# m-dayani/EORB_SLAM

Measured on AMD Instinct MI355X. Metric: front-end frames/s (event-accumulate + extract + match) per GPU; HBM GB/s vs roofline, higher is better.
Workload: dtype f32; 1 GPU; BASELINE.json configs[1]: synthetic 1000000 events/slice on 240x180 (shapes generator, DAVIS sensor pixels; raw (x,y,t,p) records resolved on the GPU through the calibrator's undistortion maps built from the EvETHZ intrinsics, as the reference loader does on the CPU), ev2im_gauss sigma=1 -> ORB-1000 (1.2, 4 levels, FAST 10/0, edge 19) -> SearchForInitialization vs previous slice; input=raw, sequences_per_gpu=1, parallelism=1 GPU

## Files before the change

### eorb_slam_amd/csrc/ev_slots.hip

```cpp
#include "eorb_ctx.h"
#include "ev_common.h"
#include "dev_math.h"
#include "sl_hot_asm.h"
#include <algorithm>
#include <memory>
#include <stdlib.h>
#include <string.h>
#include <vector>

namespace eorb {

constexpr uint32_t kNoSlot = 0xffu;
typedef uint16_t slot_entry;
constexpr uint32_t kEntryTag = 0x1000u;
constexpr int kSlotScatWaves = 8;
constexpr uint16_t kNoGeo = 0xffffu;
constexpr int kCountWaves = 16;

__global__ void sl_assign_kernel(const uint32_t* __restrict__ src_info, int nsrc, int W, int H, int h, int TX,
                                 uint32_t* __restrict__ tile_nslots, uint2* __restrict__ slot_tab, uint16_t* __restrict__ slot_geo,
                                 int* __restrict__ info)
{
    const int i = blockIdx.x * blockDim.x + threadIdx.x;
    if (i >= nsrc) { if (i == nsrc) slot_geo[i] = kNoGeo; return; }
// ... 258 lines not shown
                                const int t = (ty0 + dy) * TX + tx0 + dx;
                                const uint32_t o = atomicAdd(&cnt[t >> 1], 1u << (16 * (t & 1)));
                                rk |= (uint64_t)((o >> (16 * (t & 1))) & 0xfffu) << (12 * j);
                            }
                        }
                    }
                    const int k = k0 + u * 64;
                    if (k < cd.n) ((uint64_t*)rec16)[cd.start + k] = (uint64_t)(r16[u] & 0xffffu) | (rk << 16);
                }
                continue;
            }
#pragma unroll
            for (int u = 0; u < U; u++) {
                if (g[u] != kNoGeo) {
                    const int t0 = (int)((g[u] >> 7) & 0x7f) * TX + (int)(g[u] & 0x7f);
                    const bool two_x = (g[u] >> 14) & 1, two_y = (g[u] >> 15) & 1;
                    atomicAdd(&cnt[t0 >> 1], 1u << (16 * (t0 & 1)));
                    if (two_x) atomicAdd(&cnt[(t0 + 1) >> 1], 1u << (16 * ((t0 + 1) & 1)));
                    if (two_y) {
                        atomicAdd(&cnt[(t0 + TX) >> 1], 1u << (16 * ((t0 + TX) & 1)));
                        if (two_x) atomicAdd(&cnt[(t0 + TX + 1) >> 1], 1u << (16 * ((t0 + TX + 1) & 1)));
                    }
                }
            }
        }
        __builtin_amdgcn_wave_barrier();
        uint16_t* sc = segcnt + (size_t)ch * NT;
        const uint16_t* c16 = (const uint16_t*)cnt;
        for (int i = lane; i < NT; i += 64) sc[i] = c16[i];
        __builtin_amdgcn_wave_barrier();
    }
}

__global__ __launch_bounds__(1024) void sl_scan_kernel(const int* __restrict__ slice_chunk0, const uint16_t* __restrict__ segcnt, int NT,
                                                       uint32_t* __restrict__ segbase, uint32_t* __restrict__ tile_cnt,
                                                       uint32_t* __restrict__ tile_base)
{
    __shared__ uint32_t wsum[16];
    __shared__ uint32_t carry;
    const int slice = blockIdx.x;
    const int c0 = slice_chunk0[slice], c1 = slice_chunk0[slice + 1];
    const int lane = threadIdx.x & 63, wave = threadIdx.x >> 6;
    if (threadIdx.x == 0) carry = 0;
    __syncthreads();
    for (int t0 = 0; t0 < NT; t0 += blockDim.x) {
        const int tile = t0 + threadIdx.x;
        uint32_t run = 0;
        if (tile < NT) {
            int c = c0;
            for (; c + 8 <= c1; c += 8) {
                uint32_t v[8];
#pragma unroll
                for (int u = 0; u < 8; u++) v[u] = segcnt[(size_t)(c + u) * NT + tile];
#pragma unroll
                for (int u = 0; u < 8; u++) { segbase[(size_t)(c + u) * NT + tile] = run; run += v[u]; }
            }
            for (; c < c1; c++) { const uint32_t v = segcnt[(size_t)c * NT + tile]; segbase[(size_t)c * NT + tile] = run; run += v; }
            tile_cnt[(size_t)slice * NT + tile] = run;
        }
        const uint32_t padded = (run + 15u) & ~15u;
        uint32_t incl = (uint32_t)wave_incl_scan((int)padded);
        if (lane == 63) wsum[wave] = incl;
        __syncthreads();
        uint32_t before = carry;
        for (int w = 0; w < wave; w++) before += wsum[w];
        if (tile < NT) tile_base[(size_t)slice * NT + tile] = before + incl - padded;
        __syncthreads();
        if (threadIdx.x == blockDim.x - 1) carry = before + incl;
        __syncthreads();
    }
}

__global__ __launch_bounds__(64 * kSlotScatWaves) void sl_scatter_kernel(const eorb_raw_event* __restrict__ ev, const ChunkDesc* __restrict__ chunks,
                                                                         const uint2* __restrict__ slot_tab, int stride, int LW, int LH, int TX, int TY,
                                                                         int NT, int chunk_cap, const int64_t* __restrict__ slice_ebase,
                                                                         const uint32_t* __restrict__ segbase, const uint32_t* __restrict__ tile_base,
                                                                         slot_entry* __restrict__ entries)
{
    extern __shared__ unsigned char sm2[];
    __shared__ uint32_t s_wsum[kSlotScatWaves];
    constexpr int NTHR = 64 * kSlotScatWaves;
    constexpr int R = 2;
    const int tid = threadIdx.x, lane = tid & 63, wave = tid >> 6;
    const int chunk = blockIdx.x;
    const ChunkDesc cd = chunks[chunk];
    const int NTp = (NT + 1) & ~1;
    uint32_t* pay = (uint32_t*)sm2;
    uint16_t* prng = (uint16_t*)(pay + chunk_cap);
    uint16_t* sidx = prng + chunk_cap;
    uint16_t* cntw = sidx + (size_t)chunk_cap * R * R;
    uint16_t* loff = cntw + kSlotScatWaves * NTp;
    uint32_t* gbase = (uint32_t*)(loff + NTp + 2);
// ... 881 lines not shown
            const int g = std::min(ncu, (nchunks + kCountWaves - 1) / kCountWaves);
            static const int tc_env = [] { const char* e = getenv("EORB_SLOT_TRANSCODE"); return e ? atoi(e) : 1; }();
            uint16_t* d_rec16 = nullptr;
            static const int pre_env = [] { const char* e = getenv("EORB_SLOT_PRERANK"); return e ? atoi(e) : 1; }();
            const int pre_on = c->dbg_slot_prerank >= 0 ? c->dbg_slot_prerank : pre_env;
            if (pre_on && (stride == 16 || stride == 4 || stride == 2) && nsrc <= 65535 && sc.rank && sl_lds_pre(NT, chunk) <= 158 * 1024) {
                if ((rc = ensure(c, ws.rec16, sizeof(uint64_t) * (size_t)std::max<int64_t>(h_offsets[B], 1)))) return rc;
                d_rec16 = (uint16_t*)ws.rec16.p;
                prerank = true;
#define SL_COUNTR(ST, BIT) do { if ((rc = sl_optin(c, BIT, (const void*)sl_count_lds_kernel<ST, false, true>, 159 * 1024))) return rc; \
                sl_count_lds_kernel<ST, false, true><<<g, 64 * kCountWaves, lds_c, M>>>(d_ev, d_chunks, nchunks, d_geo, c->lut_w, c->lut_h, TX, NT, d_segcnt, SlotDict{nullptr, 0u, nullptr, nullptr, 0}, d_rec16); } while (0)
                if (stride == 16) SL_COUNTR(16, 18); else if (stride == 4) SL_COUNTR(4, 19); else SL_COUNTR(2, 20);
#undef SL_COUNTR
            }
            else {
            if (tc_env && stride == 16 && nsrc <= 65535 && sc.rank) {
                if ((rc = ensure(c, ws.rec16, sizeof(uint16_t) * (size_t)std::max<int64_t>(h_offsets[B], 1)))) return rc;
                d_rec16 = (uint16_t*)ws.rec16.p;
            }
#define SL_COUNT(ST, BIT) do { if ((rc = sl_optin(c, BIT, (const void*)sl_count_lds_kernel<ST>, 159 * 1024))) return rc; \
                sl_count_lds_kernel<ST><<<g, 64 * kCountWaves, lds_c, M>>>(d_ev, d_chunks, nchunks, d_geo, c->lut_w, c->lut_h, TX, NT, d_segcnt, SlotDict{nullptr, 0u, nullptr, nullptr}, d_rec16); } while (0)
            if (stride == 16) SL_COUNT(16, 0); else if (stride == 4) SL_COUNT(4, 1); else if (stride == 2) SL_COUNT(2, 10); else SL_COUNT(-4, 2);
#undef SL_COUNT
            if (d_rec16) { d_ev = (const eorb_raw_event*)d_rec16; scat_stride = 2; }
            }
        }
        else if (nchunks) {
            if (stride == 16) sl_count_kernel<16><<<nchunks, 256, lds, M>>>(d_ev, d_chunks, d_tab, c->lut_w, c->lut_h, TX, NT, d_segcnt);
            else if (stride == 4) sl_count_kernel<4><<<nchunks, 256, lds, M>>>(d_ev, d_chunks, d_tab, c->lut_w, c->lut_h, TX, NT, d_segcnt);
            else if (stride == 2) sl_count_kernel<2><<<nchunks, 256, lds, M>>>(d_ev, d_chunks, d_tab, c->lut_w, c->lut_h, TX, NT, d_segcnt);
            else sl_count_kernel<-4><<<nchunks, 256, lds, M>>>(d_ev, d_chunks, d_tab, c->lut_w, c->lut_h, TX, NT, d_segcnt);
        }
        ps.reset(); ps.reset(new ProfScope(c, "ev_scan"));
        sl_scan_kernel<<<B, 1024, 0, M>>>(d_slice_c0, d_segcnt, NT, d_segbase, d_tile_cnt, d_tile_base);
        ps.reset();
        EORB_HIP(c, hipEventRecord(E[0], M));
        EORB_HIP(c, hipStreamWaitEvent(P, E[0], 0));
        EORB_HIP(c, hipMemsetAsync(ws.hot.p, 0, 256, P));
        sl_plan_kernel<<<NT, 256, sizeof(uint32_t) * 2 * (size_t)B, P>>>(d_tile_cnt, d_tile_base, d_slice_eb, B, NT, TX, hot_min, d_nslots, d_rowbase,
                                                                               d_items, d_tile_w, d_tile_m, d_ctr, d_hot_cnt, d_hot_items, hot_cap);
        sl_tasks_kernel<<<1, 1024, sizeof(uint32_t) * (size_t)NT, P>>>(d_tile_w, d_tile_m, NT, Gt, max_per_tile, d_scr, d_task, d_hot_cnt, hot_cap);
        EORB_HIP(c, hipEventRecord(E[1], P));
        ProfScope ps2(c, "ev_scatter");
        const int stride = scat_stride;
        if (nchunks && prerank) {
            const size_t lds_p = sl_lds_pre(NT, chunk);
            const uint16_t* d_segcnt_c = d_segcnt;
            if (sc.waves == 16) {
                if ((rc = sl_optin(c, 16, (const void*)sl_scatter_pre_kernel<16>, 159 * 1024))) return rc;
                sl_scatter_pre_kernel<16><<<nchunks, 64 * 16, lds_p, M>>>((const uint64_t*)ws.rec16.p, d_chunks, d_tab, c->lut_w * c->lut_h, TX, NT, chunk, d_slice_eb, d_segcnt_c, d_segbase, d_tile_base, (slot_entry*)ws.entries.p);
            } else {
                if ((rc = sl_optin(c, 17, (const void*)sl_scatter_pre_kernel<8>, 159 * 1024))) return rc;
                sl_scatter_pre_kernel<8><<<nchunks, 64 * 8, lds_p, M>>>((const uint64_t*)ws.rec16.p, d_chunks, d_tab, c->lut_w * c->lut_h, TX, NT, chunk, d_slice_eb, d_segcnt_c, d_segbase, d_tile_base, (slot_entry*)ws.entries.p);
            }
        }
        else if (nchunks && sc.rank) {
#define SL_SCAT(ST, NW, BIT) do { if ((rc = sl_optin(c, BIT, (const void*)sl_scatter_rank_kernel<ST, NW>, 159 * 1024))) return rc; \
                sl_scatter_rank_kernel<ST, NW><<<nchunks, 64 * NW, sc.lds, M>>>(d_ev, d_chunks, d_tab, c->lut_w, c->lut_h, TX, NT, chunk, \
                                                                                   d_slice_eb, d_segbase, d_tile_base, (slot_entry*)ws.entries.p); } while (0)
            if (sc.waves == 16) { if (stride == 16) SL_SCAT(16, 16, 3); else if (stride == 4) SL_SCAT(4, 16, 4); else if (stride == 2) SL_SCAT(2, 16, 11); else SL_SCAT(-4, 16, 5); }
            else { if (stride == 16) SL_SCAT(16, 8, 6); else if (stride == 4) SL_SCAT(4, 8, 7); else if (stride == 2) SL_SCAT(2, 8, 12); else SL_SCAT(-4, 8, 8); }
#undef SL_SCAT
        }
        else if (nchunks)
            sl_scatter_kernel<<<nchunks, 64 * kSlotScatWaves, sc.lds, M>>>(d_ev, d_chunks, d_tab, stride, c->lut_w, c->lut_h, TX, TY, NT, chunk,
                                                                                 d_slice_eb, d_segbase, d_tile_base, (slot_entry*)ws.entries.p);
        EORB_LAUNCH_CHECK(c, "ev_bin (slot) kernels");
// ... 77 lines not shown
```

### eorb_slam_amd/csrc/orb_extract.hip

```cpp
#include "eorb_ctx.h"
#include "dev_math.h"
#include "orb_pattern.h"
#include <math.h>
#include <algorithm>
#include <string.h>
#include <vector>

namespace eorb {

struct DevGeom {
    LevelGeom lv[kMaxLevels];
    int nlevels, edge, W, H;
    int pyr_bytes, roi_bytes, ncells, cell_cap, cand_total, kp_total, max_out;
    int iniTh, minTh;
    int umax[16];
    float sf[kMaxLevels];
    int oct_in_lds[2][7], oct_off[2][7];
    int oct_lds_bytes[2], oct_gblock_bytes[2];
    int oct_dyn[2], oct_off_dyn[2][7], oct_dyn_base[2], oct_dyn_lds[2];
    int oct_direct_cap[2];
    int node_cap_max, vsp_cap_max, ncap_max;
};

__device__ __constant__ signed char c_pattern[1024];
// ... 53 lines not shown
    }
}

__global__ void pyr_resize_kernel(int level, const DevGeom* __restrict__ G, const short4* __restrict__ tabs,
                                  uint8_t* __restrict__ pyr)
{
    const LevelGeom& L = G->lv[level];
    const LevelGeom& P = G->lv[level - 1];
    const int slice = blockIdx.y;
    uint8_t* base = pyr + (size_t)slice * G->pyr_bytes;
    const uint8_t* sroi = base + P.buf_off + (size_t)G->edge * P.bw + G->edge;
    uint8_t* dst = base + L.buf_off;
    const short4* xt = tabs + L.xtab_off;
    const short4* yt = tabs + L.ytab_off;
    const int n = L.bw * L.bh;
    for (int i = blockIdx.x * blockDim.x + threadIdx.x; i < n; i += gridDim.x * blockDim.x) {
        const int y = i / L.bw, x = i - y * L.bw;
        const int dy = reflect101(y - G->edge, L.h), dx = reflect101(x - G->edge, L.w);
        const short4 xc = xt[dx], yc = yt[dy];
        const uint8_t* S0 = sroi + (size_t)yc.x * P.bw;
        const uint8_t* S1 = sroi + (size_t)yc.y * P.bw;
        int r0, r1;
        if (dx < L.xmax) {
            r0 = S0[xc.x] * xc.y + S0[xc.x + 1] * xc.z;
            r1 = S1[xc.x] * xc.y + S1[xc.x + 1] * xc.z;
        } else {
            r0 = S0[xc.x] * 2048;
            r1 = S1[xc.x] * 2048;
        }
        dst[i] = (uint8_t)((((yc.z * (r0 >> 4)) >> 16) + ((yc.w * (r1 >> 4)) >> 16) + 2) >> 2);
    }
}

__device__ __forceinline__ int fast_S(const uint8_t* __restrict__ t, int pitch)
{
    const int v = t[0];
    int d[16];
    d[0] = v - t[3 * pitch];          d[1] = v - t[3 * pitch + 1];   d[2] = v - t[2 * pitch + 2];   d[3] = v - t[pitch + 3];
    d[4] = v - t[3];                  d[5] = v - t[-pitch + 3];      d[6] = v - t[-2 * pitch + 2];  d[7] = v - t[-3 * pitch + 1];
    d[8] = v - t[-3 * pitch];         d[9] = v - t[-3 * pitch - 1];  d[10] = v - t[-2 * pitch - 2]; d[11] = v - t[-pitch - 3];
    d[12] = v - t[-3];                d[13] = v - t[pitch - 3];      d[14] = v - t[2 * pitch - 2];  d[15] = v - t[3 * pitch - 1];
    int mn2[16], mx2[16], mn4[16], mx4[16], mn8[16], mx8[16];
#pragma unroll
    for (int k = 0; k < 16; k++) { mn2[k] = min(d[k], d[(k + 1) & 15]); mx2[k] = max(d[k], d[(k + 1) & 15]); }
#pragma unroll
    for (int k = 0; k < 16; k++) { mn4[k] = min(mn2[k], mn2[(k + 2) & 15]); mx4[k] = max(mx2[k], mx2[(k + 2) & 15]); }
#pragma unroll
    for (int k = 0; k < 16; k++) { mn8[k] = min(mn4[k], mn4[(k + 4) & 15]); mx8[k] = max(mx4[k], mx4[(k + 4) & 15]); }
    int A = -256, Bm = 256;
#pragma unroll
    for (int k = 0; k < 16; k++) {
        A = max(A, min(mn8[k], d[(k + 8) & 15]));
        Bm = min(Bm, max(mx8[k], d[(k + 8) & 15]));
    }
    return max(A, -Bm);
}

constexpr int kCellMax = 60;

__global__ __launch_bounds__(256) void fast_cells_kernel(const DevGeom* __restrict__ G, const uint8_t* __restrict__ pyr,
                                                         int32_t* __restrict__ cell_cnt, uint32_t* __restrict__ cell_cand)
{
    __shared__ uint8_t tile[(kCellMax + 6) * (kCellMax + 8)];
    __shared__ uint8_t smap[(kCellMax + 2) * (kCellMax + 2)];
    __shared__ uint8_t s_cnt[16 * 4];
    const int slice = blockIdx.y;
    int cid = blockIdx.x, level = 0;
    while (level + 1 < G->nlevels && cid >= G->lv[level + 1].cell_off) level++;
    const LevelGeom& L = G->lv[level];
    const int local = cid - L.cell_off;
    const int ci = local / L.nCols, cj = local - ci * L.nCols;
    const int tid = threadIdx.x;
    int32_t* out_cnt = cell_cnt + (size_t)slice * G->ncells + cid;
    uint32_t* out = cell_cand + ((size_t)slice * G->ncells + cid) * G->cell_cap;
    const int iniY = L.minBY + ci * L.hCell, iniX = L.minBX + cj * L.wCell;
    int maxY = iniY + L.hCell + 6, maxX = iniX + L.wCell + 6;
    if (iniY >= L.maxBY - 3 || iniX >= L.maxBX - 3) { if (tid == 0) *out_cnt = 0; return; }
    maxY = min(maxY, L.maxBY); maxX = min(maxX, L.maxBX);
    const int cw = maxX - iniX, ch = maxY - iniY;
    const int dw = cw - 6, dh = ch - 6;
    if (dw <= 0 || dh <= 0) { if (tid == 0) *out_cnt = 0; return; }
    const uint8_t* roi = pyr + (size_t)slice * G->pyr_bytes + L.buf_off + (size_t)G->edge * L.bw + G->edge;
    const int pitch = kCellMax + 8;
    const uint8_t first = roi[(size_t)iniY * L.bw + iniX];
    int differs = 0;
    for (int i = tid; i < cw * ch; i += 256) {
        const int y = i / cw, x = i - y * cw;
        const uint8_t v = roi[(size_t)(iniY + y) * L.bw + iniX + x];
        tile[y * pitch + x] = v;
        differs |= (v != first);
    }
    if (!__syncthreads_or(differs) && G->iniTh >= 0 && G->minTh >= 0) { if (tid == 0) *out_cnt = 0; return; }
    const int sp = dw + 2;
    for (int i = tid; i < (dw + 2) * (dh + 2); i += 256) smap[i] = 0;
    __syncthreads();
    for (int i = tid; i < dw * dh; i += 256) {
        const int y = i / dw, x = i - y * dw;
        int S = fast_S(&tile[(y + 3) * pitch + x + 3], pitch);
        smap[(y + 1) * sp + x + 1] = (uint8_t)min(max(S, 0), 255);
    }
    __syncthreads();
    int th = G->iniTh;
    const int npix = dw * dh, npass = (npix + 255) / 256;
    const int w = tid >> 6, lane = tid & 63;
    for (int attempt = 0; attempt < 2; attempt++) {
        uint32_t flags = 0u;
        for (int p = 0; p < npass; p++) {
            const int i = p * 256 + tid;
            bool kp = false;
            if (i < npix) {
                const int y = i / dw, x = i - y * dw;
                const uint8_t* c = &smap[(y + 1) * sp + x + 1];
                const int S = c[0];
                if (S > th) {
                    const int sc = S - 1;
                    kp = true;
#pragma unroll
                    for (int oy = -1; oy <= 1; oy++)
#pragma unroll
                        for (int ox = -1; ox <= 1; ox++) {
                            if (ox == 0 && oy == 0) continue;
                            const int Sn = c[oy * sp + ox];
                            const int scn = (Sn > th) ? Sn - 1 : 0;
                            kp = kp && (sc > scn);
                        }
                }
            }
            const uint64_t bal = __ballot(kp);
            if (kp) flags |= 1u << p;
            if (lane == 0) s_cnt[p * 4 + w] = (uint8_t)__popcll(bal);
        }
        __syncthreads();
        int run = 0;
        for (int p = 0; p < npass; p++) {
            const int c0 = s_cnt[p * 4 + 0], c1 = s_cnt[p * 4 + 1], c2 = s_cnt[p * 4 + 2], c3 = s_cnt[p * 4 + 3];
            const bool kp = (flags >> p) & 1u;
            const uint64_t bal = __ballot(kp);
            if (kp) {
                const int base = run + (w > 0 ? c0 : 0) + (w > 1 ? c1 : 0) + (w > 2 ? c2 : 0);
                const int pos = base + __popcll(bal & ((lane == 0) ? 0ull : (~0ull >> (64 - lane))));
                const int i = p * 256 + tid, y = i / dw, x = i - y * dw;
                const int S = smap[(y + 1) * sp + x + 1];
                const uint32_t kx = (uint32_t)(x + 3 + cj * L.wCell), ky = (uint32_t)(y + 3 + ci * L.hCell);
                if (pos < G->cell_cap) out[pos] = kx | (ky << 12) | ((uint32_t)(S - 1) << 24);
            }
            run += c0 + c1 + c2 + c3;
        }
        if (run > 0 || th == G->minTh) { if (tid == 0) *out_cnt = min(run, G->cell_cap); break; }
        th = G->minTh;
        if (attempt == 1 && tid == 0) *out_cnt = 0;
        __syncthreads();
    }
}

struct ONode { uint16_t x0, x1, y0, y1, start, cnt, seq; uint8_t flags, pad; };
static_assert(sizeof(ONode) == 16, "ONode is 16 bytes");
constexpr int kOctThreads = 512;
constexpr int kOctBigNode = 1024;
constexpr int kOctBigMax = 64;

__device__ __forceinline__ int oct_wave_incl_scan(int x)
{
    x += __builtin_amdgcn_update_dpp(0, x, 0x111, 0xf, 0xf, false);
    x += __builtin_amdgcn_update_dpp(0, x, 0x112, 0xf, 0xf, false);
    x += __builtin_amdgcn_update_dpp(0, x, 0x114, 0xf, 0xf, false);
    x += __builtin_amdgcn_update_dpp(0, x, 0x118, 0xf, 0xf, false);
    x += __builtin_amdgcn_update_dpp(0, x, 0x142, 0xa, 0xf, false);
    x += __builtin_amdgcn_update_dpp(0, x, 0x143, 0xc, 0xf, false);
    return x;
}

__device__ int oct_block_scan(int* a, int n, int* ws)
{
    const int tid = threadIdx.x, lane = tid & 63, wave = tid >> 6, nw = blockDim.x >> 6;
// ... 779 lines not shown
{
    const int slice = blockIdx.y;
    const int gid = blockIdx.x * 8 + (threadIdx.x >> 5);
    const int u = (int)(threadIdx.x & 31) - 15;
    if (gid >= G->kp_total) return;
    int level = 0;
    while (level + 1 < G->nlevels && gid >= G->lv[level + 1].kp_off) level++;
    const LevelGeom& L = G->lv[level];
    const int i = gid - L.kp_off;
    if (i >= lvl_cnt[slice * G->nlevels + level]) return;
    const uint32_t p = lvl_kp[(size_t)slice * G->kp_total + gid];
    const int cx = (int)(p & 0xfff) + L.minBX, cy = (int)((p >> 12) & 0xfff) + L.minBY;
    const uint8_t* center = pyr + (size_t)slice * G->pyr_bytes + L.buf_off + (size_t)(cy + G->edge) * L.bw + (cx + G->edge);
    const int step = L.bw;
    const int au = u < 0 ? -u : u;
    int m_01 = 0, m_10 = 0;
    if (au <= 15) m_10 = u * (int)center[u];
#pragma unroll
    for (int v = 1; v <= 15; ++v) {
        if (au <= G->umax[v]) {
            const int val_plus = center[u + v * step], val_minus = center[u - v * step];
            m_01 += v * (val_plus - val_minus);
            m_10 += u * (val_plus + val_minus);
        }
    }
#pragma unroll
    for (int d = 16; d >= 1; d >>= 1) {
        m_01 += __shfl_xor(m_01, d, 64);
        m_10 += __shfl_xor(m_10, d, 64);
    }
    if ((threadIdx.x & 31) == 0) kp_angle[(size_t)slice * G->kp_total + gid] = dev_fast_atan2((float)m_01, (float)m_10);
}

constexpr int kBlurTW = 64, kBlurTH = 16;
__global__ __launch_bounds__(256) void blur_kernel(const DevGeom* __restrict__ G, const uint8_t* __restrict__ pyr,
                                                   uint8_t* __restrict__ blur)
{
    __shared__ int rows[(kBlurTH + 4) * kBlurTW];
    const int slice = blockIdx.z;
    int level = 0, ty = blockIdx.y;
    while (level < G->nlevels) {
        const int nty = (G->lv[level].h + kBlurTH - 1) / kBlurTH;
        if (ty < nty) break;
        ty -= nty; level++;
    }
    if (level >= G->nlevels) return;
    const LevelGeom& L = G->lv[level];
    const int x0 = blockIdx.x * kBlurTW, y0 = ty * kBlurTH;
    if (x0 >= L.w) return;
    const uint8_t* roi = pyr + (size_t)slice * G->pyr_bytes + L.buf_off + (size_t)G->edge * L.bw + G->edge;
    const int k0 = 39, k1 = 57, k2 = 64;
    for (int i = threadIdx.x; i < (kBlurTH + 4) * kBlurTW; i += 256) {
        const int r = i / kBlurTW, cxi = i - r * kBlurTW;
        const int sy = reflect101(y0 + r - 2, L.h);
        const int x = x0 + cxi;
        int acc = 0;
        if (x < L.w) {
            const uint8_t* Srow = roi + (size_t)sy * L.bw;
            acc = k0 * Srow[reflect101(x - 2, L.w)] + k1 * Srow[reflect101(x - 1, L.w)] + k2 * Srow[x] +
                  k1 * Srow[reflect101(x + 1, L.w)] + k0 * Srow[reflect101(x + 2, L.w)];
        }
        rows[i] = acc;
    }
    __syncthreads();
    for (int i = threadIdx.x; i < kBlurTH * kBlurTW; i += 256) {
        const int ly = i / kBlurTW, lx = i - ly * kBlurTW;
        const int x = x0 + lx, y = y0 + ly;
        if (x < L.w && y < L.h) {
            const int acc = k0 * rows[(ly + 0) * kBlurTW + lx] + k1 * rows[(ly + 1) * kBlurTW + lx] + k2 * rows[(ly + 2) * kBlurTW + lx] +
                            k1 * rows[(ly + 3) * kBlurTW + lx] + k0 * rows[(ly + 4) * kBlurTW + lx];
            int v = (acc + (1 << 15)) >> 16;
            v = min(max(v, 0), 255);
            blur[(size_t)slice * G->roi_bytes + L.roi_off + (size_t)y * L.w + x] = (uint8_t)v;
        }
    }
}

__device__ __forceinline__ int brief_byte(const uint8_t* __restrict__ img, int w, int h, int cx, int cy, float angle_deg, int b, int& oob)
{
    const float factorPI = (float)(3.1415926535897932384626433832795 / 180.f);
    const float angle = angle_deg * factorPI;
    float sb, ca;
    dev_sincosf(angle, &sb, &ca);
    const float a = ca, bb = sb;
    const int step = w;
    const int base = cy * step + cx;
    const int total = w * h;
    const signed char* pat = c_pattern + b * 32;
    int val = 0;
#pragma unroll
    for (int k = 0; k < 8; k++) {
        int t[2];
#pragma unroll
        for (int s = 0; s < 2; s++) {
            const float px = (float)pat[(2 * k + s) * 2], py = (float)pat[(2 * k + s) * 2 + 1];
            const float r0 = px * bb, r1 = py * a;
            const float c0 = px * a, c1 = py * bb;
            const int dy = dev_cvround(r0 + r1);
            const int dx = dev_cvround(c0 - c1);
            const int idx = base + dy * step + dx;
            if (idx < 0 || idx >= total) { oob = 1; t[s] = 0; }
            else t[s] = img[idx];
        }
        val |= (t[0] < t[1]) << k;
    }
    return val;
// ... 423 lines not shown
            const int n = o.lv[l].bw * o.lv[l].bh;
            pyr_resize_kernel<<<dim3(B >= 16 ? (n + 1023) / 1024 : (n + 255) / 256, B), 256, 0, c->stream>>>(l, G, (const short4*)o.tabs.p, pyr);
        }
        EORB_LAUNCH_CHECK(c, "pyramid kernels");
    }
    {
        ProfScope ps(c, "orb_fast_cells");
        fast_cells_kernel<<<dim3(o.ncells, B), 256, 0, c->stream>>>(G, pyr, (int32_t*)c->cell_cnt.p, (uint32_t*)c->cell_cand.p);
        EORB_LAUNCH_CHECK(c, "fast_cells_kernel");
    }
    {
        ProfScope ps(c, "orb_octree");
        int32_t* sticky = d_flag_out ? nullptr : (int32_t*)c->status.p;
        int32_t* redo = err_flag + 16;
        if (o.oct_all_lds[placement])
            octree_kernel<true><<<B * o.nlevels, kOctThreads, o.oct_lds[placement], c->stream>>>(G, (const int32_t*)c->cell_cnt.p, (const uint32_t*)c->cell_cand.p,
                                                                    (unsigned char*)c->oct_scratch.p, (uint32_t*)c->lvl_kp.p, (int32_t*)c->lvl_cnt.p, err_flag, sticky, placement, nullptr);
        else if (o.oct_dyn[placement]) {
            octree_kernel<true><<<B * o.nlevels, kOctThreads, o.oct_dyn_lds[placement], c->stream>>>(G, (const int32_t*)c->cell_cnt.p, (const uint32_t*)c->cell_cand.p,
                                                                    (unsigned char*)c->oct_scratch.p, (uint32_t*)c->lvl_kp.p, (int32_t*)c->lvl_cnt.p, err_flag, sticky, placement, redo);
            octree_kernel<false><<<B * o.nlevels, kOctThreads, o.oct_lds[placement], c->stream>>>(G, (const int32_t*)c->cell_cnt.p, (const uint32_t*)c->cell_cand.p,
                                                                    (unsigned char*)c->oct_scratch.p, (uint32_t*)c->lvl_kp.p, (int32_t*)c->lvl_cnt.p, err_flag, sticky, placement, redo);
        } else
            octree_kernel<false><<<B * o.nlevels, kOctThreads, o.oct_lds[placement], c->stream>>>(G, (const int32_t*)c->cell_cnt.p, (const uint32_t*)c->cell_cand.p,
                                                                    (unsigned char*)c->oct_scratch.p, (uint32_t*)c->lvl_kp.p, (int32_t*)c->lvl_cnt.p, err_flag, sticky, placement, nullptr);
        EORB_LAUNCH_CHECK(c, "octree_kernel");
    }
    static const int fuse_env = [] { const char* e = getenv("EORB_ORB_DESCRIBE"); return e ? atoi(e) : 1; }();
    const bool none_in = (float)lap1 < (float)o.lv[0].minBX, all_in = lap0 <= 0 && lap1 >= o.W;
    const bool one_launch = fuse_env != 0 && !c->dbg_orb_three_launches && (none_in || all_in);
    const int all_stereo = !none_in && all_in;
    if (want_desc) {
        ProfScope ps(c, "orb_blur");
        int tyt = 0, wmax = 0;
        for (int l = 0; l < o.nlevels; l++) { tyt += (o.lv[l].h + kBlurTH - 1) / kBlurTH; wmax = std::max(wmax, o.lv[l].w); }
        blur_kernel<<<dim3((wmax + kBlurTW - 1) / kBlurTW, tyt, B), 256, 0, c->stream>>>(G, pyr, (uint8_t*)c->blur.p);
        EORB_LAUNCH_CHECK(c, "blur_kernel");
    }
    if (one_launch) {
        ProfScope ps(c, "orb_describe");
        const dim3 grid((o.kp_total + 7) / 8, B);
        if (want_desc)
            describe_kernel<true><<<grid, 256, 0, c->stream>>>(G, pyr, (const uint8_t*)c->blur.p, (const uint32_t*)c->lvl_kp.p, (const int32_t*)c->lvl_cnt.p,
                                                              all_stereo, o.max_out, d_kps, d_desc, d_oob, d_n, d_mono, err_flag, d_flag_out);
        else
            describe_kernel<false><<<grid, 256, 0, c->stream>>>(G, pyr, nullptr, (const uint32_t*)c->lvl_kp.p, (const int32_t*)c->lvl_cnt.p,
                                                               all_stereo, o.max_out, d_kps, d_desc, d_oob, d_n, d_mono, err_flag, d_flag_out);
        EORB_LAUNCH_CHECK(c, "describe_kernel");
        return EORB_OK;
    }
    {
        ProfScope ps(c, "orb_orient");
        orient_kernel<<<dim3((o.kp_total + 7) / 8, B), 256, 0, c->stream>>>(G, pyr, (const uint32_t*)c->lvl_kp.p,
                                                                              (const int32_t*)c->lvl_cnt.p, (float*)c->kp_angle.p);
        EORB_LAUNCH_CHECK(c, "orient_kernel");
    }
    if (want_desc) {
        ProfScope ps(c, "orb_brief");
        brief_kernel<<<dim3((o.kp_total + 7) / 8, B), 256, 0, c->stream>>>(G, (const uint8_t*)c->blur.p, (const uint32_t*)c->lvl_kp.p,
                                                                           (const int32_t*)c->lvl_cnt.p, (const float*)c->kp_angle.p,
                                                                           (uint8_t*)c->out_desc.p, (uint8_t*)c->out_oob.p);
        EORB_LAUNCH_CHECK(c, "brief_kernel");
    }
    {
        ProfScope ps(c, "orb_assemble");
        assemble_kernel<<<B, 256, 0, c->stream>>>(G, (const uint32_t*)c->lvl_kp.p, (const int32_t*)c->lvl_cnt.p,
                                                  (const float*)c->kp_angle.p, (const uint8_t*)c->out_desc.p,
                                                  (const uint8_t*)c->out_oob.p, lap0, lap1, want_desc, o.max_out, d_kps, d_desc,
                                                  d_oob, d_n, d_mono, err_flag, d_flag_out);
// ... 39 lines not shown
        if (!out) return EORB_OK;
        if (cap_bytes < total * 3 * sizeof(float))
            return set_err(c, EORB_E_ARG, "debug_stage: 'cand' of level %d needs %zu bytes, %zu given", level, total * 3 * sizeof(float), cap_bytes);
        float* rec = (float*)out;
        for (int i = 0; i < nc; i++) {
            const int n = std::min(std::max(cnt[i], 0), o.cell_cap);
            for (int k = 0; k < n; k++) {
                const uint32_t v = cand[(size_t)i * o.cell_cap + k];
                *rec++ = (float)(v & 0xfffu); *rec++ = (float)((v >> 12) & 0xfffu); *rec++ = (float)(v >> 24);
            }
        }
        return EORB_OK;
    }
    return set_err(c, EORB_E_ARG, "debug_stage: stage '%s' unknown (pyr, blur, cand)", name);
}

int orb_pyramid_blur_dev(eorb_ctx* c, const uint8_t* d_img, int img_stride)
{
    OrbState& o = c->orb;
    if (!o.configured) return set_err(c, EORB_E_NOTCONF, "orb: eorb_orb_configure not called");
    int rc;
    if ((rc = ensure(c, c->pyr, (size_t)o.pyr_bytes))) return rc;
    if ((rc = ensure(c, c->blur, (size_t)o.roi_bytes))) return rc;
    const DevGeom* G = (const DevGeom*)o.geom.p;
    uint8_t* pyr = (uint8_t*)c->pyr.p;
    o.last_B = 1; o.last_blur = true; o.last_cells = false;
    ProfScope ps(c, "orb_pyr_blur");
    const int n0 = o.lv[0].bw * o.lv[0].bh;
    pyr_level0_kernel<<<dim3((n0 + 255) / 256, 1), 256, 0, c->stream>>>(d_img, img_stride, 0, G, pyr, nullptr);
    for (int l = 1; l < o.nlevels; l++) {
        const int n = o.lv[l].bw * o.lv[l].bh;
        pyr_resize_kernel<<<dim3((n + 255) / 256, 1), 256, 0, c->stream>>>(l, G, (const short4*)o.tabs.p, pyr);
    }
    int tyt = 0, wmax = 0;
    for (int l = 0; l < o.nlevels; l++) { tyt += (o.lv[l].h + kBlurTH - 1) / kBlurTH; wmax = std::max(wmax, o.lv[l].w); }
    blur_kernel<<<dim3((wmax + kBlurTW - 1) / kBlurTW, tyt, 1), 256, 0, c->stream>>>(G, pyr, (uint8_t*)c->blur.p);
    EORB_LAUNCH_CHECK(c, "pyramid/blur kernels");
    return EORB_OK;
}

int orb_tracked_dev(eorb_ctx* c, eorb_keypoint* d_kps, int n, int mode, const uint8_t* d_ref, uint8_t* d_desc, uint8_t* d_oob)
{
    if (n <= 0) return EORB_OK;
    OrbState& o = c->orb;
    ProfScope ps(c, "orb_tracked_desc");
    tracked_desc_kernel<<<(n + 7) / 8, 256, 0, c->stream>>>((const DevGeom*)o.geom.p, (const uint8_t*)c->blur.p, d_kps, n, mode,
                                                           d_ref, d_desc, d_oob);
    EORB_LAUNCH_CHECK(c, "tracked_desc_kernel");
    return EORB_OK;
}

__global__ __launch_bounds__(256) void stereo_match_kernel(const DevGeom* __restrict__ G, const uint8_t* __restrict__ pyr, const eorb_keypoint* __restrict__ kps,
                                                           const uint8_t* __restrict__ desc, const int32_t* __restrict__ n, int cap, float mb, float mbf,
                                                           float* __restrict__ uRight, float* __restrict__ depth, int32_t* __restrict__ sad)
{
    const int lane = threadIdx.x & 63;
    const int iL = blockIdx.x * 4 + (threadIdx.x >> 6);
    const int N = min(n[0], cap), Nr = min(n[1], cap);
    if (iL >= N) return;
    const eorb_keypoint kL = kps[iL];
    const eorb_keypoint* kR = kps + cap;
    const uint64_t* dR = (const uint64_t*)(desc + (size_t)cap * 32);
    const uint64_t* dl = (const uint64_t*)(desc + (size_t)iL * 32);
    const uint64_t d0 = dl[0], d1 = dl[1], d2 = dl[2], d3 = dl[3];
    if (lane == 0) { uRight[iL] = -1.0f; depth[iL] = -1.0f; sad[iL] = -1; }
    const int levelL = kL.octave;
    const float vL = kL.y, uL = kL.x;
    const int row = (int)vL;
    const float minD = 0.f, maxD = mbf / mb;
// ... 146 lines not shown
```

Before: 47240 frames/s.

## Parallelize slot scan across tiles and vectorize FAST scoring and Gaussian blur

The per-slice chunk scan, previously one block per slice walking every chunk serially, is split into a grid over tile groups and 16 chunk segments per block that combine partial sums in LDS. The tile-base prefix now runs as a separate small kernel. FAST scoring computes two pixels per thread with packed 16-bit min/max on word-aligned LDS reads, and index division is replaced by incremental raster stepping. The blur kernel processes four pixels per thread with packed row sums, flattens the tile grid so empty tiles are not launched, and uses taller tiles. The cost is an extra kernel launch and more complex indexing.

```diff
diff --git a/eorb_slam_amd/csrc/ev_slots.hip b/eorb_slam_amd/csrc/ev_slots.hip
--- a/eorb_slam_amd/csrc/ev_slots.hip
+++ b/eorb_slam_amd/csrc/ev_slots.hip
@@ -314,32 +314,59 @@
     }
 }
 
-__global__ __launch_bounds__(1024) void sl_scan_kernel(const int* __restrict__ slice_chunk0, const uint16_t* __restrict__ segcnt, int NT,
-                                                       uint32_t* __restrict__ segbase, uint32_t* __restrict__ tile_cnt,
-                                                       uint32_t* __restrict__ tile_base)
+constexpr int kScanSegs = 16, kScanTrip = 16;
+__global__ __launch_bounds__(64 * kScanSegs) void sl_scan_kernel(const int* __restrict__ slice_chunk0, const uint16_t* __restrict__ segcnt, int NT,
+                                                                 uint32_t* __restrict__ segbase, uint32_t* __restrict__ tile_cnt)
+{
+    __shared__ uint32_t part[kScanSegs][64];
+    const int slice = blockIdx.y;
+    const int c0 = slice_chunk0[slice], c1 = slice_chunk0[slice + 1];
+    const int lane = threadIdx.x & 63, seg = threadIdx.x >> 6;
+    const int tile = blockIdx.x * 64 + lane;
+    const int len = (c1 - c0 + kScanSegs - 1) / kScanSegs;
+    const int s0 = min(c0 + seg * len, c1), s1 = min(s0 + len, c1);
+    const bool live = tile < NT;
+    uint32_t v[kScanTrip];
+    uint32_t sum = 0;
+    for (int c = s0; c < s1; c += kScanTrip) {
+#pragma unroll
+        for (int u = 0; u < kScanTrip; u++) v[u] = (live && c + u < s1) ? segcnt[(size_t)(c + u) * NT + tile] : 0u;
+#pragma unroll
+        for (int u = 0; u < kScanTrip; u++) sum += v[u];
+    }
+    part[seg][lane] = sum;
+    __syncthreads();
+    uint32_t run = 0, total = 0;
+#pragma unroll
+    for (int s = 0; s < kScanSegs; s++) { const uint32_t p = part[s][lane]; run += s < seg ? p : 0u; total += p; }
+    if (!live) return;
+    if (seg == 0) tile_cnt[(size_t)slice * NT + tile] = total;
+    if (len <= kScanTrip) {
+#pragma unroll
+        for (int u = 0; u < kScanTrip; u++)
+            if (s0 + u < s1) { segbase[(size_t)(s0 + u) * NT + tile] = run; run += v[u]; }
+        return;
+    }
+    for (int c = s0; c < s1; c += kScanTrip) {
+#pragma unroll
+        for (int u = 0; u < kScanTrip; u++) v[u] = c + u < s1 ? segcnt[(size_t)(c + u) * NT + tile] : 0u;
+#pragma unroll
+        for (int u = 0; u < kScanTrip; u++)
+            if (c + u < s1) { segbase[(size_t)(c + u) * NT + tile] = run; run += v[u]; }
+    }
+}
+
+__global__ __launch_bounds__(1024) void sl_tile_base_kernel(const uint32_t* __restrict__ tile_cnt, int NT, uint32_t* __restrict__ tile_base)
 {
     __shared__ uint32_t wsum[16];
     __shared__ uint32_t carry;
     const int slice = blockIdx.x;
-    const int c0 = slice_chunk0[slice], c1 = slice_chunk0[slice + 1];
     const int lane = threadIdx.x & 63, wave = threadIdx.x >> 6;
     if (threadIdx.x == 0) carry = 0;
     __syncthreads();
     for (int t0 = 0; t0 < NT; t0 += blockDim.x) {
         const int tile = t0 + threadIdx.x;
-        uint32_t run = 0;
-        if (tile < NT) {
-            int c = c0;
-            for (; c + 8 <= c1; c += 8) {
-                uint32_t v[8];
-#pragma unroll
-                for (int u = 0; u < 8; u++) v[u] = segcnt[(size_t)(c + u) * NT + tile];
-#pragma unroll
-                for (int u = 0; u < 8; u++) { segbase[(size_t)(c + u) * NT + tile] = run; run += v[u]; }
-            }
-            for (; c < c1; c++) { const uint32_t v = segcnt[(size_t)c * NT + tile]; segbase[(size_t)c * NT + tile] = run; run += v; }
-            tile_cnt[(size_t)slice * NT + tile] = run;
-        }
+        const uint32_t run = tile < NT ? tile_cnt[(size_t)slice * NT + tile] : 0u;
         const uint32_t padded = (run + 15u) & ~15u;
         uint32_t incl = (uint32_t)wave_incl_scan((int)padded);
         if (lane == 63) wsum[wave] = incl;
@@ -1287,7 +1314,8 @@
             else sl_count_kernel<-4><<<nchunks, 256, lds, M>>>(d_ev, d_chunks, d_tab, c->lut_w, c->lut_h, TX, NT, d_segcnt);
         }
         ps.reset(); ps.reset(new ProfScope(c, "ev_scan"));
-        sl_scan_kernel<<<B, 1024, 0, M>>>(d_slice_c0, d_segcnt, NT, d_segbase, d_tile_cnt, d_tile_base);
+        sl_scan_kernel<<<dim3((NT + 63) / 64, B), 64 * kScanSegs, 0, M>>>(d_slice_c0, d_segcnt, NT, d_segbase, d_tile_cnt);
+        sl_tile_base_kernel<<<B, 1024, 0, M>>>(d_tile_cnt, NT, d_tile_base);
         ps.reset();
         EORB_HIP(c, hipEventRecord(E[0], M));
         EORB_HIP(c, hipStreamWaitEvent(P, E[0], 0));
diff --git a/eorb_slam_amd/csrc/orb_extract.hip b/eorb_slam_amd/csrc/orb_extract.hip
--- a/eorb_slam_amd/csrc/orb_extract.hip
+++ b/eorb_slam_amd/csrc/orb_extract.hip
@@ -109,38 +109,60 @@
     }
 }
 
-__device__ __forceinline__ int fast_S(const uint8_t* __restrict__ t, int pitch)
-{
-    const int v = t[0];
-    int d[16];
-    d[0] = v - t[3 * pitch];          d[1] = v - t[3 * pitch + 1];   d[2] = v - t[2 * pitch + 2];   d[3] = v - t[pitch + 3];
-    d[4] = v - t[3];                  d[5] = v - t[-pitch + 3];      d[6] = v - t[-2 * pitch + 2];  d[7] = v - t[-3 * pitch + 1];
-    d[8] = v - t[-3 * pitch];         d[9] = v - t[-3 * pitch - 1];  d[10] = v - t[-2 * pitch - 2]; d[11] = v - t[-pitch - 3];
-    d[12] = v - t[-3];                d[13] = v - t[pitch - 3];      d[14] = v - t[2 * pitch - 2];  d[15] = v - t[3 * pitch - 1];
-    int mn2[16], mx2[16], mn4[16], mx4[16], mn8[16], mx8[16];
-#pragma unroll
-    for (int k = 0; k < 16; k++) { mn2[k] = min(d[k], d[(k + 1) & 15]); mx2[k] = max(d[k], d[(k + 1) & 15]); }
-#pragma unroll
-    for (int k = 0; k < 16; k++) { mn4[k] = min(mn2[k], mn2[(k + 2) & 15]); mx4[k] = max(mx2[k], mx2[(k + 2) & 15]); }
-#pragma unroll
-    for (int k = 0; k < 16; k++) { mn8[k] = min(mn4[k], mn4[(k + 4) & 15]); mx8[k] = max(mx4[k], mx4[(k + 4) & 15]); }
-    int A = -256, Bm = 256;
+typedef short short2v __attribute__((ext_vector_type(2)));
+__device__ __forceinline__ short2v pk_min(short2v a, short2v b) { return __builtin_elementwise_min(a, b); }
+__device__ __forceinline__ short2v pk_max(short2v a, short2v b) { return __builtin_elementwise_max(a, b); }
+#define FAST_PAIR(r, k) __builtin_bit_cast(short2v, __builtin_amdgcn_perm(hi[r], lo[r], 0x0c000c00u | (uint32_t)(k) | ((uint32_t)((k) + 1) << 16)))
+__device__ __forceinline__ short2v fast_S2(const uint32_t* __restrict__ tile32, int pitch32, int row, int x)
+{
+    uint32_t lo[7], hi[7];
+    const uint32_t* t = tile32 + row * pitch32 + ((x + 1) >> 2);
+    const uint32_t sh = (uint32_t)(x + 1) & 3u;
+#pragma unroll
+    for (int r = 0; r < 7; r++) {
+        const uint32_t d0 = t[r * pitch32], d1 = t[r * pitch32 + 1], d2 = t[r * pitch32 + 2];
+        lo[r] = __builtin_amdgcn_alignbyte(d1, d0, sh);
+        hi[r] = __builtin_amdgcn_alignbyte(d2, d1, sh);
+    }
+    const short2v v = FAST_PAIR(3, 3);
+    short2v d[16];
+    d[0] = v - FAST_PAIR(6, 3);   d[1] = v - FAST_PAIR(6, 4);   d[2] = v - FAST_PAIR(5, 5);   d[3] = v - FAST_PAIR(4, 6);
+    d[4] = v - FAST_PAIR(3, 6);   d[5] = v - FAST_PAIR(2, 6);   d[6] = v - FAST_PAIR(1, 5);   d[7] = v - FAST_PAIR(0, 4);
+    d[8] = v - FAST_PAIR(0, 3);   d[9] = v - FAST_PAIR(0, 2);   d[10] = v - FAST_PAIR(1, 1);  d[11] = v - FAST_PAIR(2, 0);
+    d[12] = v - FAST_PAIR(3, 0);  d[13] = v - FAST_PAIR(4, 0);  d[14] = v - FAST_PAIR(5, 1);  d[15] = v - FAST_PAIR(6, 2);
+    short2v mn2[16], mx2[16], mn4[16], mx4[16], mn8[16], mx8[16];
+#pragma unroll
+    for (int k = 0; k < 16; k++) { mn2[k] = pk_min(d[k], d[(k + 1) & 15]); mx2[k] = pk_max(d[k], d[(k + 1) & 15]); }
+#pragma unroll
+    for (int k = 0; k < 16; k++) { mn4[k] = pk_min(mn2[k], mn2[(k + 2) & 15]); mx4[k] = pk_max(mx2[k], mx2[(k + 2) & 15]); }
+#pragma unroll
+    for (int k = 0; k < 16; k++) { mn8[k] = pk_min(mn4[k], mn4[(k + 4) & 15]); mx8[k] = pk_max(mx4[k], mx4[(k + 4) & 15]); }
+    short2v A = (short2v)(-256), Bm = (short2v)(256);
 #pragma unroll
     for (int k = 0; k < 16; k++) {
-        A = max(A, min(mn8[k], d[(k + 8) & 15]));
-        Bm = min(Bm, max(mx8[k], d[(k + 8) & 15]));
-    }
-    return max(A, -Bm);
-}
+        A = pk_max(A, pk_min(mn8[k], d[(k + 8) & 15]));
+        Bm = pk_min(Bm, pk_max(mx8[k], d[(k + 8) & 15]));
+    }
+    return pk_max(A, (short2v)(0) - Bm);
+}
+#undef FAST_PAIR
 
 constexpr int kCellMax = 60;
+constexpr int kCellPitch = 72;
+
+struct RasterPos {
+    int y, x, w, qs, rs;
+    __device__ __forceinline__ RasterPos(int i, int w_) : w(w_) { y = i / w; x = i - y * w; qs = 256 / w; rs = 256 - qs * w; }
+    __device__ __forceinline__ void step() { x += rs; y += qs; if (x >= w) { x -= w; y++; } }
+};
 
 __global__ __launch_bounds__(256) void fast_cells_kernel(const DevGeom* __restrict__ G, const uint8_t* __restrict__ pyr,
                                                          int32_t* __restrict__ cell_cnt, uint32_t* __restrict__ cell_cand)
 {
-    __shared__ uint8_t tile[(kCellMax + 6) * (kCellMax + 8)];
+    __shared__ uint32_t tile32[(kCellMax + 6) * kCellPitch / 4];
     __shared__ uint8_t smap[(kCellMax + 2) * (kCellMax + 2)];
     __shared__ uint8_t s_cnt[16 * 4];
+    uint8_t* tile = (uint8_t*)tile32;
     const int slice = blockIdx.y;
     int cid = blockIdx.x, level = 0;
     while (level + 1 < G->nlevels && cid >= G->lv[level + 1].cell_off) level++;
@@ -158,36 +180,45 @@
     const int dw = cw - 6, dh = ch - 6;
     if (dw <= 0 || dh <= 0) { if (tid == 0) *out_cnt = 0; return; }
     const uint8_t* roi = pyr + (size_t)slice * G->pyr_bytes + L.buf_off + (size_t)G->edge * L.bw + G->edge;
-    const int pitch = kCellMax + 8;
     const uint8_t first = roi[(size_t)iniY * L.bw + iniX];
     int differs = 0;
-    for (int i = tid; i < cw * ch; i += 256) {
-        const int y = i / cw, x = i - y * cw;
-        const uint8_t v = roi[(size_t)(iniY + y) * L.bw + iniX + x];
-        tile[y * pitch + x] = v;
-        differs |= (v != first);
+    {
+        RasterPos q(tid, cw);
+        for (int i = tid; i < cw * ch; i += 256, q.step()) {
+            const uint8_t v = roi[(size_t)(iniY + q.y) * L.bw + iniX + q.x];
+            tile[q.y * kCellPitch + q.x + 1] = v;
+            differs |= (v != first);
+        }
     }
     if (!__syncthreads_or(differs) && G->iniTh >= 0 && G->minTh >= 0) { if (tid == 0) *out_cnt = 0; return; }
     const int sp = dw + 2;
     for (int i = tid; i < (dw + 2) * (dh + 2); i += 256) smap[i] = 0;
     __syncthreads();
-    for (int i = tid; i < dw * dh; i += 256) {
-        const int y = i / dw, x = i - y * dw;
-        int S = fast_S(&tile[(y + 3) * pitch + x + 3], pitch);
-        smap[(y + 1) * sp + x + 1] = (uint8_t)min(max(S, 0), 255);
+    {
+        const int pw = (dw + 1) >> 1;
+        RasterPos q(tid, pw);
+        for (int i = tid; i < pw * dh; i += 256, q.step()) {
+            const int x = 2 * q.x;
+            short2v S = fast_S2(tile32, kCellPitch / 4, q.y, x);
+            S = pk_min(pk_max(S, (short2v)(0)), (short2v)(255));
+            uint8_t* o = &smap[(q.y + 1) * sp + x + 1];
+            o[0] = (uint8_t)S.x;
+            if (x + 1 < dw) o[1] = (uint8_t)S.y;
+        }
     }
     __syncthreads();
     int th = G->iniTh;
     const int npix = dw * dh, npass = (npix + 255) / 256;
     const int w = tid >> 6, lane = tid & 63;
+    const RasterPos q0(tid, dw);
     for (int attempt = 0; attempt < 2; attempt++) {
         uint32_t flags = 0u;
-        for (int p = 0; p < npass; p++) {
+        RasterPos q = q0;
+        for (int p = 0; p < npass; p++, q.step()) {
             const int i = p * 256 + tid;
             bool kp = false;
             if (i < npix) {
-                const int y = i / dw, x = i - y * dw;
-                const uint8_t* c = &smap[(y + 1) * sp + x + 1];
+                const uint8_t* c = &smap[(q.y + 1) * sp + q.x + 1];
                 const int S = c[0];
                 if (S > th) {
                     const int sc = S - 1;
@@ -209,14 +240,15 @@
         }
         __syncthreads();
         int run = 0;
-        for (int p = 0; p < npass; p++) {
+        q = q0;
+        for (int p = 0; p < npass; p++, q.step()) {
             const int c0 = s_cnt[p * 4 + 0], c1 = s_cnt[p * 4 + 1], c2 = s_cnt[p * 4 + 2], c3 = s_cnt[p * 4 + 3];
             const bool kp = (flags >> p) & 1u;
             const uint64_t bal = __ballot(kp);
             if (kp) {
                 const int base = run + (w > 0 ? c0 : 0) + (w > 1 ? c1 : 0) + (w > 2 ? c2 : 0);
                 const int pos = base + __popcll(bal & ((lane == 0) ? 0ull : (~0ull >> (64 - lane))));
-                const int i = p * 256 + tid, y = i / dw, x = i - y * dw;
+                const int y = q.y, x = q.x;
                 const int S = smap[(y + 1) * sp + x + 1];
                 const uint32_t kx = (uint32_t)(x + 3 + cj * L.wCell), ky = (uint32_t)(y + 3 + ci * L.hCell);
                 if (pos < G->cell_cap) out[pos] = kx | (ky << 12) | ((uint32_t)(S - 1) << 24);
@@ -1062,46 +1094,68 @@
     if ((threadIdx.x & 31) == 0) kp_angle[(size_t)slice * G->kp_total + gid] = dev_fast_atan2((float)m_01, (float)m_10);
 }
 
-constexpr int kBlurTW = 64, kBlurTH = 16;
+constexpr int kBlurTW = 64, kBlurTH = 28;
+static int blur_tiles(const OrbState& o)
+{
+    int n = 0;
+    for (int l = 0; l < o.nlevels; l++) n += ((o.lv[l].w + kBlurTW - 1) / kBlurTW) * ((o.lv[l].h + kBlurTH - 1) / kBlurTH);
+    return n;
+}
 __global__ __launch_bounds__(256) void blur_kernel(const DevGeom* __restrict__ G, const uint8_t* __restrict__ pyr,
                                                    uint8_t* __restrict__ blur)
 {
-    __shared__ int rows[(kBlurTH + 4) * kBlurTW];
-    const int slice = blockIdx.z;
-    int level = 0, ty = blockIdx.y;
-    while (level < G->nlevels) {
-        const int nty = (G->lv[level].h + kBlurTH - 1) / kBlurTH;
-        if (ty < nty) break;
-        ty -= nty; level++;
-    }
-    if (level >= G->nlevels) return;
+    __shared__ uint2 rows[(kBlurTH + 4) * (kBlurTW / 4)];
+    const int slice = blockIdx.y;
+    int level = 0, t = blockIdx.x, ntx = 1;
+    for (;; level++) {
+        if (level >= G->nlevels) return;
+        ntx = (G->lv[level].w + kBlurTW - 1) / kBlurTW;
+        const int nt = ntx * ((G->lv[level].h + kBlurTH - 1) / kBlurTH);
+        if (t < nt) break;
+        t -= nt;
+    }
     const LevelGeom& L = G->lv[level];
-    const int x0 = blockIdx.x * kBlurTW, y0 = ty * kBlurTH;
-    if (x0 >= L.w) return;
-    const uint8_t* roi = pyr + (size_t)slice * G->pyr_bytes + L.buf_off + (size_t)G->edge * L.bw + G->edge;
+    const int ty = t / ntx, tx = t - ty * ntx;
+    const int x0 = tx * kBlurTW, y0 = ty * kBlurTH;
+    const int E = G->edge;
+    const uint32_t* lvl = (const uint32_t*)(pyr + (size_t)slice * G->pyr_bytes + L.buf_off);
+    const int q = threadIdx.x & 15, x = x0 + 4 * q;
     const int k0 = 39, k1 = 57, k2 = 64;
-    for (int i = threadIdx.x; i < (kBlurTH + 4) * kBlurTW; i += 256) {
-        const int r = i / kBlurTW, cxi = i - r * kBlurTW;
-        const int sy = reflect101(y0 + r - 2, L.h);
-        const int x = x0 + cxi;
-        int acc = 0;
-        if (x < L.w) {
-            const uint8_t* Srow = roi + (size_t)sy * L.bw;
-            acc = k0 * Srow[reflect101(x - 2, L.w)] + k1 * Srow[reflect101(x - 1, L.w)] + k2 * Srow[x] +
-                  k1 * Srow[reflect101(x + 1, L.w)] + k0 * Srow[reflect101(x + 2, L.w)];
-        }
-        rows[i] = acc;
+    for (int r = threadIdx.x >> 4; r < kBlurTH + 4; r += 16) {
+        const int y = y0 + r - 2;
+        if (x < L.w && y <= L.h + 1) {
+            const int o = (y + E) * L.bw + E + x - 2;
+            const uint32_t* p = lvl + (o >> 2);
+            const uint32_t d0 = p[0], d1 = p[1], d2 = p[2];
+            const uint32_t lo = __builtin_amdgcn_alignbyte(d1, d0, (uint32_t)o & 3u), hi = __builtin_amdgcn_alignbyte(d2, d1, (uint32_t)o & 3u);
+            const int b0 = lo & 0xff, b1 = (lo >> 8) & 0xff, b2 = (lo >> 16) & 0xff, b3 = lo >> 24;
+            const int b4 = hi & 0xff, b5 = (hi >> 8) & 0xff, b6 = (hi >> 16) & 0xff, b7 = hi >> 24;
+            const uint32_t s0 = k0 * (b0 + b4) + k1 * (b1 + b3) + k2 * b2, s1 = k0 * (b1 + b5) + k1 * (b2 + b4) + k2 * b3;
+            const uint32_t s2 = k0 * (b2 + b6) + k1 * (b3 + b5) + k2 * b4, s3 = k0 * (b3 + b7) + k1 * (b4 + b6) + k2 * b5;
+            rows[r * (kBlurTW / 4) + q] = make_uint2(s0 | (s1 << 16), s2 | (s3 << 16));
+        }
     }
     __syncthreads();
-    for (int i = threadIdx.x; i < kBlurTH * kBlurTW; i += 256) {
-        const int ly = i / kBlurTW, lx = i - ly * kBlurTW;
-        const int x = x0 + lx, y = y0 + ly;
+    for (int ly = threadIdx.x >> 4; ly < kBlurTH; ly += 16) {
+        const int y = y0 + ly;
         if (x < L.w && y < L.h) {
-            const int acc = k0 * rows[(ly + 0) * kBlurTW + lx] + k1 * rows[(ly + 1) * kBlurTW + lx] + k2 * rows[(ly + 2) * kBlurTW + lx] +
-                            k1 * rows[(ly + 3) * kBlurTW + lx] + k0 * rows[(ly + 4) * kBlurTW + lx];
-            int v = (acc + (1 << 15)) >> 16;
-            v = min(max(v, 0), 255);
-            blur[(size_t)slice * G->roi_bytes + L.roi_off + (size_t)y * L.w + x] = (uint8_t)v;
+            uint2 v[5];
+#pragma unroll
+            for (int k = 0; k < 5; k++) v[k] = rows[(ly + k) * (kBlurTW / 4) + q];
+            uint32_t out = 0;
+#pragma unroll
+            for (int j = 0; j < 4; j++) {
+                int a[5];
+#pragma unroll
+                for (int k = 0; k < 5; k++) a[k] = (int)(((j < 2 ? v[k].x : v[k].y) >> (16 * (j & 1))) & 0xffffu);
+                const int acc = k0 * (a[0] + a[4]) + k1 * (a[1] + a[3]) + k2 * a[2];
+                int r8 = (acc + (1 << 15)) >> 16;
+                r8 = min(max(r8, 0), 255);
+                out |= (uint32_t)r8 << (8 * j);
+            }
+            uint8_t* dst = blur + (size_t)slice * G->roi_bytes + L.roi_off + (size_t)y * L.w + x;
+            if (x + 3 < L.w) __builtin_memcpy(dst, &out, 4);
+            else for (int j = 0; x + j < L.w; j++) dst[j] = (uint8_t)(out >> (8 * j));
         }
     }
 }
@@ -1591,9 +1645,7 @@
     const int all_stereo = !none_in && all_in;
     if (want_desc) {
         ProfScope ps(c, "orb_blur");
-        int tyt = 0, wmax = 0;
-        for (int l = 0; l < o.nlevels; l++) { tyt += (o.lv[l].h + kBlurTH - 1) / kBlurTH; wmax = std::max(wmax, o.lv[l].w); }
-        blur_kernel<<<dim3((wmax + kBlurTW - 1) / kBlurTW, tyt, B), 256, 0, c->stream>>>(G, pyr, (uint8_t*)c->blur.p);
+        blur_kernel<<<dim3(blur_tiles(o), B), 256, 0, c->stream>>>(G, pyr, (uint8_t*)c->blur.p);
         EORB_LAUNCH_CHECK(c, "blur_kernel");
     }
     if (one_launch) {
@@ -1699,9 +1751,7 @@
         const int n = o.lv[l].bw * o.lv[l].bh;
         pyr_resize_kernel<<<dim3((n + 255) / 256, 1), 256, 0, c->stream>>>(l, G, (const short4*)o.tabs.p, pyr);
     }
-    int tyt = 0, wmax = 0;
-    for (int l = 0; l < o.nlevels; l++) { tyt += (o.lv[l].h + kBlurTH - 1) / kBlurTH; wmax = std::max(wmax, o.lv[l].w); }
-    blur_kernel<<<dim3((wmax + kBlurTW - 1) / kBlurTW, tyt, 1), 256, 0, c->stream>>>(G, pyr, (uint8_t*)c->blur.p);
+    blur_kernel<<<dim3(blur_tiles(o), 1), 256, 0, c->stream>>>(G, pyr, (uint8_t*)c->blur.p);
     EORB_LAUNCH_CHECK(c, "pyramid/blur kernels");
     return EORB_OK;
 }
```

Measured after the change: 47900 frames/s (median of 6 runs). 1.01x the previous value.
